# gardiens/EOGS2

Measured on AMD Instinct MI355X. Metric: rasterizer fwd+bwd throughput @1M Gaussians/1024^2 (train iters/s with 1 render/iter), higher is better.
Workload: dtype f32; 1 GPU; 1048576 Gaussians x 1024x1024 x 5 channels, opacity=init, 1 view per GPU, fwd+bwd; gaussians=1048576, height=1024, width=1024, num_rendered=4236528, list_entries=1681274, list_block_px=8, parallelism=view-dp1

## Files before the change

eogs2_amd/csrc/common.h:

```cpp
#pragma once
#include <hip/hip_runtime.h>
#include <stdint.h>
#include <stddef.h>
#include <stdlib.h>

#include "eogs_rast.h"
#include "eogs_loss.h"
#include "eogs_optim.h"
#include "eogs_resample.h"
#include "eogs_knn.h"
#include "eogs_shade.h"
#include "eogs_reg.h"
#include "eogs_pan.h"
#include "eogs_density.h"
#include "eogs_step.h"
#include "eogs_monitor.h"
#include "eogs_tsdf.h"
#include "eogs_dsm.h"

#define NCH EOGS_RAST_CHANNELS
#define TILE EOGS_RAST_TILE
#define SUBX 8
#define SUBY 8
#define PPL (SUBX * SUBY / 64)
// ... 131 lines not shown
#define EOGS_DEPTH_SWITCH 0
#define MACRO_KEY_BITS 16
static_assert(BLOCK_BIG * BLOCK_BIG <= 16, "the sub-mask lives in the upper 16 bits of the sort key");

template <int MACRO, class Emit>
__device__ inline void walk_macro_row(uint32_t kind, unsigned long long m, const SpanParams& sp, int sx0, int sy0, int sx1,
                                      int sy1, int MY, Emit&& emit) {
  const int sw = sx1 - sx0;
  int c0[MACRO], c1[MACRO];
  unsigned long long w[MACRO];
  int lo = 0x7FFFFFFF, hi = -1;
#pragma unroll
  for (int dy = 0; dy < MACRO; dy++) {
    const int fy = MY * MACRO + dy;
    c0[dy] = c1[dy] = 0;
    w[dy] = 0ull;
    if (fy < sy0 || fy >= sy1) continue;
    if (kind == BK_MASK) {
      w[dy] = (m >> ((fy - sy0) * sw)) & (sw >= 64 ? ~0ull : ((1ull << sw) - 1ull));
      if (w[dy]) {
        lo = min(lo, sx0 + (int)__builtin_ctzll(w[dy]));
        hi = max(hi, sx0 + 63 - (int)__builtin_clzll(w[dy]));
      }
    } else {
      if (kind == BK_SPANS) row_span(sp, fy, sx0, sx1, c0[dy], c1[dy]);
      else { c0[dy] = sx0; c1[dy] = sx1; }
      if (c1[dy] > c0[dy]) {
        lo = min(lo, c0[dy]);
        hi = max(hi, c1[dy] - 1);
      }
    }
  }
  if (hi < 0) return;
  for (int MX = lo / MACRO; MX <= hi / MACRO; MX++) {
    const int X0 = MX * MACRO;
    uint32_t sub = 0;
#pragma unroll
    for (int dy = 0; dy < MACRO; dy++) {
      uint32_t nib;
      if (kind == BK_MASK) {
        const int off = X0 - sx0;
        nib = (uint32_t)((off >= 0 ? (w[dy] >> off) : (w[dy] << (-off))) & ((1ull << MACRO) - 1ull));
      } else {
        const int a = max(c0[dy], X0) - X0, b = min(c1[dy], X0 + MACRO) - X0;
        nib = b > a ? (((1u << (b - a)) - 1u) << a) : 0u;
      }
      sub |= nib << (dy * MACRO);
    }
    if (sub) emit(MX, sub);
  }
}

template <int MACRO>
__device__ inline void count_macro_row(uint32_t kind, const SpanParams& sp, int sx0, int sy0, int sx1, int sy1, int MY,
                                       uint32_t& ent, uint32_t& fine) {
  int c0[MACRO], c1[MACRO];
  int lo = 0x7FFFFFFF, hi = -1;
#pragma unroll
  for (int dy = 0; dy < MACRO; dy++) {
    const int fy = MY * MACRO + dy;
    c0[dy] = c1[dy] = 0;
    if (fy < sy0 || fy >= sy1) continue;
    if (kind == BK_SPANS) row_span(sp, fy, sx0, sx1, c0[dy], c1[dy]);
    else { c0[dy] = sx0; c1[dy] = sx1; }
    if (c1[dy] > c0[dy]) {
      lo = min(lo, c0[dy]);
      hi = max(hi, c1[dy] - 1);
    }
  }
  if (hi < 0) return;
  const int B0 = lo / MACRO, B1 = hi / MACRO;
  if (B1 - B0 < 64) {
    unsigned long long m = 0ull;
#pragma unroll
    for (int dy = 0; dy < MACRO; dy++) {
      if (c1[dy] > c0[dy]) {
        const int a = c0[dy] / MACRO - B0, len = (c1[dy] - 1) / MACRO - c0[dy] / MACRO + 1;
        m |= (len >= 64 ? ~0ull : ((1ull << len) - 1ull)) << a;
        fine += (uint32_t)(c1[dy] - c0[dy]);
      }
    }
    ent += (uint32_t)__popcll(m);
  } else {
    walk_macro_row<MACRO>(kind, 0ull, sp, sx0, sy0, sx1, sy1, MY, [&](int, uint32_t sub) {
      ent++;
      fine += (uint32_t)__popc(sub);
    });
  }
}

static inline size_t ws_align(size_t x) { return (x + 255u) & ~(size_t)255u; }

template <typename T>
static inline size_t ws_carve(char* base, size_t off, T*& p, size_t count) {
  off = ws_align(off);
  p = base ? reinterpret_cast<T*>(base + off) : nullptr;
  return off + count * sizeof(T);
}

static inline uint32_t ceil_div_u32(uint64_t a, uint64_t b) { return (uint32_t)((a + b - 1) / b); }

struct GeomWS {
  float4* packed;
  uint4* binfo;
  float4* bext;
  uint32_t* pbkey;
  uint32_t* pblock;
  uint32_t* pblockE;
  uint32_t* bcount;
  uint32_t* bpairs;
  uint32_t* sched;
  uint32_t* where;
  uint32_t* misc;
  float* vmpart;
  uint32_t nblkE;
  size_t bytes;
};

static inline GeomWS geom_layout(char* base, int P) {
  GeomWS g;
  size_t n = (size_t)P, o = 0;
  g.nblkE = ceil_div_u32(n, BLK * EXPAND_ITEMS);
  o = ws_carve(base, o, g.packed, n * 4);
  o = ws_carve(base, o, g.binfo, n * 2);
  o = ws_carve(base, o, g.bext, n * 2);
  o = ws_carve(base, o, g.pblock, (size_t)g.nblkE + 1);
  o = ws_carve(base, o, g.pblockE, (size_t)g.nblkE + 1);
  o = ws_carve(base, o, g.pbkey, (size_t)g.nblkE * 4);
  o = ws_carve(base, o, g.bcount, (size_t)MAX_BLOCKS);
  o = ws_carve(base, o, g.bpairs, (size_t)MAX_BLOCKS);
  o = ws_carve(base, o, g.sched, (size_t)16);
  o = ws_carve(base, o, g.where, (size_t)3 * SCHED_MAX_BLOCKS);
  o = ws_carve(base, o, g.misc, MISC_WORDS);
  o = ws_carve(base, o, g.vmpart, (size_t)g.nblkE * 18);
  g.bytes = ws_align(o) + 256;
  return g;
}

struct SortWS {
  uint4* entA;
  uint4* entB;
  uint32_t* hist;
  uint32_t* histp;
  uint32_t* dtotal;
  uint32_t cap, nblk;
  size_t bytes;
};
static inline uint32_t ent_cap(int P) {
  const uint64_t c = 6ull * (uint64_t)(P < 0 ? 0 : P);
  return c < 4096ull ? 4096u : (c > 0x07FFFFFFull ? 0x07FFFFFFu : (uint32_t)c);
}
static inline SortWS sort_layout(char* base, uint32_t cap) {
  SortWS w;
  size_t o = 0;
  w.cap = cap;
  w.nblk = ceil_div_u32(cap, (uint64_t)SORTE_TILE);
  o = ws_carve(base, o, w.entA, (size_t)cap);
  o = ws_carve(base, o, w.entB, (size_t)cap);
  o = ws_carve(base, o, w.hist, (size_t)SORTE_MAXBINS * (w.nblk ? w.nblk : 1));
  o = ws_carve(base, o, w.histp, (size_t)SORTE_MAXBINS * (w.nblk ? w.nblk : 1));
  o = ws_carve(base, o, w.dtotal, SORTE_MAXBINS);
  w.bytes = ws_align(o) + 256;
  return w;
}

struct BinWS {
  uint2* point_list;
  uint32_t* sorted_keys;
  float* records;
  uint8_t* live;
  uint8_t* qmask;
  SortWS sort;
  int block;
  uint32_t cap_slots, cap_entries;
  size_t bytes;
};

static inline int ceil_log2_u32(uint32_t n) {
  int b = 0;
  while (((uint64_t)1 << b) < n) b++;
  return b;
}

static inline uint32_t nr_slots(int64_t R) { return (uint32_t)((uint64_t)R & 0x7FFFFFFFull); }
static inline uint32_t nr_entries(int64_t R) { return (uint32_t)(((uint64_t)R >> 32) & 0x07FFFFFFull); }
__host__ __device__ inline bool capacity_fits(uint64_t slots, uint64_t entries, uint64_t cap_slots, uint64_t cap_entries) {
  return slots <= cap_slots && entries <= cap_entries;
}
static inline int nr_alt(int64_t R) { return (int)(((uint64_t)R >> 59) & 1ull); }
static inline int nr_shallow(int64_t R) { return (int)(((uint64_t)R >> 60) & 1ull); }
static inline int nr_sorted(int64_t R) { return (int)(((uint64_t)R >> 61) & 1ull); }
static inline int nr_block(int64_t R) { return (((uint64_t)R >> 62) & 1ull) ? BLOCK_BIG : 1; }
static inline int nr_wide(int64_t R) { return (int)(((uint64_t)R >> 31) & 1ull); }
static inline int64_t nr_pack(uint32_t slots, uint32_t entries, int block, int sorted, int wide, int shallow, int alt = 0) {
  return (int64_t)(((uint64_t)(block > 1) << 62) | ((uint64_t)(sorted != 0) << 61) | ((uint64_t)(shallow != 0) << 60) |
                   ((uint64_t)(alt != 0) << 59) | ((uint64_t)(entries & 0x07FFFFFFu) << 32) | ((uint64_t)(wide != 0) << 31) | slots);
}
static inline uint32_t macro_grid_x(int W, int M) { return (uint32_t)(((W + SUBX - 1) / SUBX + M - 1) / M); }
static inline uint32_t macro_grid_y(int H, int M) { return (uint32_t)(((H + SUBY - 1) / SUBY + M - 1) / M); }
static inline void block_sort_geometry(int H, int W, int& passes, int& bits) {
  const uint32_t nb = macro_grid_x(W, BLOCK_BIG) * macro_grid_y(H, BLOCK_BIG);
  const int tb = ceil_log2_u32(nb) < 1 ? 1 : ceil_log2_u32(nb);
  passes = tb <= 12 ? 1 : 2;
  bits = (tb + passes - 1) / passes;
}

static inline BinWS bin_layout(char* base, int H, int W, int64_t R) {
  (void)H; (void)W;
  BinWS b;
  const size_t ne = (size_t)nr_entries(R), nslots = (size_t)nr_slots(R);
  size_t o = 0;
  b.block = nr_block(R);
  b.cap_slots = (uint32_t)nslots;
  b.cap_entries = (uint32_t)ne;
  o = ws_carve(base, o, b.point_list, b.block > 1 ? ne : nslots);
  o = ws_carve(base, o, b.sorted_keys, b.block > 1 ? ne : (size_t)0);
  o = ws_carve(base, o, b.records, nslots * REC);
  o = ws_carve(base, o, b.live, nslots);
  o = ws_carve(base, o, b.qmask, b.block > 1 ? (size_t)0 : nslots);
  b.sort = sort_layout(nullptr, 0);
  if (!nr_sorted(R) && ne) {
    o = ws_align(o);
    b.sort = sort_layout(base ? base + o : nullptr, (uint32_t)ne);
    o += b.sort.bytes;
  }
  b.bytes = ws_align(o) + 256;
  return b;
}

struct ImgWS {
  uint2* ranges;
  float* final_T;
  uint32_t* n_contrib;
  uint4* desc;
  uint32_t sched_lg;
  size_t bytes;
};

static inline ImgWS img_layout(char* base, int H, int W) {
  ImgWS im;
  size_t n = (size_t)H * W, o = 0;
  size_t T = (size_t)macro_grid_x(W, 1) * macro_grid_y(H, 1);
  const uint32_t nblocks = macro_grid_x(W, BLOCK_BIG) * macro_grid_y(H, BLOCK_BIG);
  o = ws_carve(base, o, im.ranges, T);
  o = ws_carve(base, o, im.final_T, n);
  o = ws_carve(base, o, im.n_contrib, n);
  im.desc = nullptr;
  im.sched_lg = 0;
  if (nblocks <= SCHED_MAX_BLOCKS && sched_enabled()) {
    im.sched_lg = sched_capacity(nblocks);
    o = ws_carve(base, o, im.desc, (size_t)8 * 16 * im.sched_lg);
  }
  im.bytes = ws_align(o) + 256;
  return im;
}

static inline char* ws_base(const void* p) {
  return reinterpret_cast<char*>((reinterpret_cast<uintptr_t>(p) + 255u) & ~(uintptr_t)255u);
}

struct FwdPrepArgs {
  int P, H, W;
  const float *means3D, *scales, *rotations, *cov3D_precomp, *opacities, *colors, *viewmatrix;
  float scale_modifier;
  bool antialiasing;
  int* radii;
  bool raw;
  const float* alt_affine;
};
void launch_preprocess_fwd(const FwdPrepArgs& a, const GeomWS& g, hipStream_t s);
void launch_pblock_scan(const GeomWS& g, int P, hipStream_t s);
void launch_entry_sort(const GeomWS& g, const SortWS& w, int P, int H, int W, hipStream_t s);
static inline bool entry_sort_result_in_A(int H, int W) {
  int passes, bits;
  block_sort_geometry(H, W, passes, bits);
  return (passes & 1) == 0;
}
void launch_block_lists(const GeomWS& g, const SortWS& w, const BinWS& b, const ImgWS& im, int P, int H, int W, int64_t R,
                        hipStream_t s);
void launch_render_fwd(const GeomWS& g, const BinWS& b, const ImgWS& im, int P, int H, int W, int64_t R,
                       const float* bg, float* out_color, float* out_invdepth, hipStream_t s);
void launch_render_bwd(const GeomWS& g, const BinWS& b, const ImgWS& im, int P, int H, int W, int64_t R,
                       const float* dL_dcolor, const float* dL_dinvdepth, const float* bg, bool raw, hipStream_t s);
int render_fwd_variant(int block, int64_t R, int P);
int render_bwd_variant(int block, int64_t R, int P);
int render_bwd_noflag_ok(int block, int64_t R, int P);
struct GaussBwdArgs {
  int P, H, W;
  const float *means3D, *scales, *rotations, *cov3D_precomp, *opacities, *viewmatrix, *projmatrix;
  const int* radii;
  float scale_modifier;
  bool antialiasing;
  float *dL_dmeans2D, *dL_dcolors, *dL_dopacity, *dL_dmeans3D, *dL_dcov3D, *dL_dscales, *dL_drotations;
  float *dL_dT_sum, *dL_dvm_mean;
  bool raw;
  const float* alt_affine;
  float* dL_dcolors_lead;
  int lead_cols;
  bool alt_only;
  int noflag_ok;
  int wide;
};
#define GB_WIDE_DEPTH 256.0f
int gaussian_bwd_wide(int64_t R, int P);
void launch_gaussian_bwd(const GaussBwdArgs& a, const GeomWS& g, const BinWS& b, int p_begin, int p_end, hipStream_t s);
void launch_selftest(uint32_t* out, hipStream_t s);

#define LOSS_WIN EOGS_LOSS_WINDOW
struct LossWindow {
  float w[LOSS_WIN];
  float ws, c1, c0;
};
struct LossWS {
  float* partial;
  float* plane_tmp;
  float* maps;
  size_t map_stride;
  int tiles;
  size_t bytes;
};
LossWS loss_layout(char* base, int planes, int H, int W, unsigned mode);
bool loss_grid_fits(int planes, int H);
void launch_loss_fwd(const LossWS& w, int planes, int H, int W, const float* img, const float* gt, unsigned mode,
                     float w_l1, float w_ssim, float bias, float* out, float* plane_sums, hipStream_t s);

void launch_sort_u32(uint32_t* keyA, uint32_t* valA, uint32_t* keyB, uint32_t* valB, uint32_t n, int passes, uint32_t* hist,
                     uint32_t nblk, uint32_t* dtotal, hipStream_t s);
```

eogs2_amd/csrc/preprocess.hip:

```cpp
#include "common.h"
#include "reduce.h"
#include <type_traits>

namespace {

struct Mat3 {
  float m[3][3];
};

__device__ inline Mat3 quat_to_Rm(float r, float x, float y, float z) {
  Mat3 R;
  R.m[0][0] = 1.f - 2.f * (y * y + z * z); R.m[1][0] = 2.f * (x * y - r * z); R.m[2][0] = 2.f * (x * z + r * y);
  R.m[0][1] = 2.f * (x * y + r * z); R.m[1][1] = 1.f - 2.f * (x * x + z * z); R.m[2][1] = 2.f * (y * z - r * x);
  R.m[0][2] = 2.f * (x * z - r * y); R.m[1][2] = 2.f * (y * z + r * x); R.m[2][2] = 1.f - 2.f * (x * x + y * y);
  return R;
}

__device__ inline void cov3d_from_scale_rot(const float s[3], float mod, const float q[4], float c6[6]) {
  Mat3 R = quat_to_Rm(q[0], q[1], q[2], q[3]);
  float sc[3] = {mod * s[0], mod * s[1], mod * s[2]};
  float M[3][3];
#pragma unroll
  for (int i = 0; i < 3; i++)
#pragma unroll
    for (int j = 0; j < 3; j++) M[i][j] = sc[i] * R.m[i][j];
  float S[3][3];
#pragma unroll
  for (int i = 0; i < 3; i++)
#pragma unroll
    for (int j = i; j < 3; j++) S[i][j] = M[0][i] * M[0][j] + M[1][i] * M[1][j] + M[2][i] * M[2][j];
  c6[0] = S[0][0]; c6[1] = S[0][1]; c6[2] = S[0][2]; c6[3] = S[1][1]; c6[4] = S[1][2]; c6[5] = S[2][2];
}

__device__ inline void build_T(const float* __restrict__ vm, int W, int H, float T[2][3]) {
  const float sx = (float)(W / 2.0), sy = (float)(H / 2.0);
#pragma unroll
  for (int k = 0; k < 3; k++) {
    T[0][k] = vm[4 * k + 0] * sx;
    T[1][k] = vm[4 * k + 1] * sy;
  }
}

__device__ inline void cov2d(const float T[2][3], const float c6[6], float& cxx, float& cxy, float& cyy) {
  const float V[3][3] = {{c6[0], c6[1], c6[2]}, {c6[1], c6[3], c6[4]}, {c6[2], c6[4], c6[5]}};
  float A[2][3];
#pragma unroll
  for (int i = 0; i < 2; i++)
#pragma unroll
    for (int l = 0; l < 3; l++) A[i][l] = T[i][0] * V[0][l] + T[i][1] * V[1][l] + T[i][2] * V[2][l];
  cxx = A[0][0] * T[0][0] + A[0][1] * T[0][1] + A[0][2] * T[0][2];
  cxy = A[1][0] * T[0][0] + A[1][1] * T[0][1] + A[1][2] * T[0][2];
  cyy = A[1][0] * T[1][0] + A[1][1] * T[1][1] + A[1][2] * T[1][2];
}

__device__ inline int clampi(int v, int lo, int hi) { return v < lo ? lo : (v > hi ? hi : v); }

__device__ inline void stage_rows3_load(const float* __restrict__ src, size_t row0, int rows, float (&r)[3]) {
  const int t = threadIdx.x, n = rows * 3;
  const float* p = src + row0 * 3;
#pragma unroll
  for (int i = 0; i < 3; i++) {
    const int e = i * BLK + t;
    r[i] = e < n ? p[e] : 0.f;
  }
}
__device__ inline void stage_rows3_store(int rows, const float (&r)[3], float* s_dst) {
  const int t = threadIdx.x, n = rows * 3;
#pragma unroll
  for (int i = 0; i < 3; i++) {
    const int e = i * BLK + t;
    if (e < n) s_dst[e] = r[i];
  }
}

constexpr float SH_C0 = 0.28209479177387814f;

__device__ inline float sigmoidf(float x) { return 1.f / (1.f + expf(-x)); }

__device__ inline float raw_activate(float s[3], float q[4], bool* clamped = nullptr) {
#pragma unroll
  for (int k = 0; k < 3; k++) s[k] = expf(s[k]);
  const float n = sqrtf(q[0] * q[0] + q[1] * q[1] + q[2] * q[2] + q[3] * q[3]);
  if (clamped) *clamped = n < 1e-12f;
  const float inv = 1.f / fmaxf(n, 1e-12f);
#pragma unroll
  for (int k = 0; k < 4; k++) q[k] *= inv;
  return inv;
}

#ifndef GB_COOP
#define GB_COOP 64u
#endif

}

#ifndef EOGS_PP_WAVES
#define EOGS_PP_WAVES 6
#endif
#define PP_ATTR __attribute__((amdgpu_waves_per_eu(EOGS_PP_WAVES, EOGS_PP_WAVES)))
template <bool RAW>
__global__ __launch_bounds__(BLK) PP_ATTR void preprocess_fwd_kernel(
    int P, int H, int W, int gx, int gy,
    const float* __restrict__ means3D, const float* __restrict__ scales, const float* __restrict__ rotations,
    const float* __restrict__ cov3D_precomp, const float* __restrict__ opacities, const float* __restrict__ colors,
    const float* __restrict__ vm, const float* __restrict__ alt, float scale_modifier, int antialiasing,
    int* __restrict__ radii, float4* __restrict__ packed, uint4* __restrict__ binfo, float4* __restrict__ bext,
    uint32_t* __restrict__ pblock,
    uint32_t* __restrict__ pbkey) {
  __shared__ float s_m[3 * BLK];
  __shared__ float s_s[3 * BLK];
  __shared__ float s_c[RAW ? 3 * BLK : 1];
  __shared__ uint32_t s_cnt[BLK / 64];
  const int t = threadIdx.x;
  const size_t row0 = (size_t)blockIdx.x * BLK;
  const int rows = (int)(((size_t)P - row0) < (size_t)BLK ? ((size_t)P - row0) : (size_t)BLK);
  float4 q_pre = make_float4(1.f, 0.f, 0.f, 0.f);
  float op_pre = 0.f;
  {
    float st_m[3], st_s[3] = {0.f, 0.f, 0.f}, st_c[3] = {0.f, 0.f, 0.f};
    stage_rows3_load(means3D, row0, rows, st_m);
    if (scales) stage_rows3_load(scales, row0, rows, st_s);
    if (RAW) stage_rows3_load(colors, row0, rows, st_c);
    if (t < rows) {
      if (!cov3D_precomp) q_pre = reinterpret_cast<const float4*>(rotations)[row0 + t];
      op_pre = opacities[row0 + t];
    }
    stage_rows3_store(rows, st_m, s_m);
    if (scales) stage_rows3_store(rows, st_s, s_s);
    if (RAW) stage_rows3_store(rows, st_c, s_c);
  }
  __syncthreads();

  const size_t idx = row0 + t;
  uint32_t my_tiles = 0, my_entries = 0, key_bits = 0, bkind = BK_RECT, my_err = 0;
  uint32_t op64 = 0;
  uint4 bi0 = make_uint4(0u, 0u, 0u, 0u);
  bool need_count = false;
  uint32_t c_kind = BK_RECT;
  SpanParams c_sp = {};
  int c_sx0 = 0, c_sy0 = 0, c_sx1 = 0, c_sy1 = 0;
  if (t < rows) {
    const float p[3] = {s_m[3 * t], s_m[3 * t + 1], s_m[3 * t + 2]};
    float pv[3];
#pragma unroll
    for (int i = 0; i < 3; i++) pv[i] = vm[i] * p[0] + vm[4 + i] * p[1] + vm[8 + i] * p[2] + vm[12 + i];

    float c6[6];
    if (cov3D_precomp) {
      const float2* c2 = reinterpret_cast<const float2*>(cov3D_precomp + 6 * idx);
      float2 a = c2[0], b = c2[1], c = c2[2];
      c6[0] = a.x; c6[1] = a.y; c6[2] = b.x; c6[3] = b.y; c6[4] = c.x; c6[5] = c.y;
    } else {
      const float4 q = q_pre;
      float s[3] = {s_s[3 * t], s_s[3 * t + 1], s_s[3 * t + 2]};
      float qq[4] = {q.x, q.y, q.z, q.w};
      if (RAW) raw_activate(s, qq);
      cov3d_from_scale_rot(s, scale_modifier, qq, c6);
    }
    float T[2][3];
    build_T(vm, W, H, T);
    float cx, cy, cz;
    cov2d(T, c6, cx, cy, cz);

    const float h_var = 0.3f;
    const float det_cov = cx * cz - cy * cy;
    cx += h_var;
    cz += h_var;
    const float det = cx * cz - cy * cy;
    float hcs = 1.0f;
    if (antialiasing) hcs = sqrtf(fmaxf(0.000025f, det_cov / det));

    int radius = 0;
    if (det != 0.0f) {
      const float det_inv = 1.f / det;
      const float mid = 0.5f * (cx + cz);
      const float root = sqrtf(fmaxf(0.1f, mid * mid - det));
      const float lambda1 = mid + root, lambda2 = mid - root;
      const float my_radius = ceilf(3.f * sqrtf(fmaxf(lambda1, lambda2)));
      const float px = (float)((((double)pv[0] + 1.0) * W - 1.0) * 0.5);
      const float py = (float)((((double)pv[1] + 1.0) * H - 1.0) * 0.5);
      const int r = (int)my_radius;
      const int x0 = clampi((int)((px - r) / TILE), 0, gx);
      const int y0 = clampi((int)((py - r) / TILE), 0, gy);
      const int x1 = clampi((int)((px + r + TILE - 1) / TILE), 0, gx);
      const int y1 = clampi((int)((py + r + TILE - 1) / TILE), 0, gy);
      const int area = (x1 - x0) * (y1 - y0);
      if (area != 0) {
        radius = r;
        const float d = (float)(200.0 - (double)pv[2]);
        if (d < 0) my_err = 0x80000000u;
        const float op_in = RAW ? sigmoidf(op_pre) : op_pre;
        const float ca = cz * det_inv, cb = -cy * det_inv, cc = cx * det_inv, op = op_in * hcs;
        op64 = (uint32_t)(fminf(fmaxf(op, 0.f), 1.f) * 64.f + 0.5f);
        const int gsx = (W + SUBX - 1) / SUBX, gsy = (H + SUBY - 1) / SUBY;
        int sx0 = FX * x0, sy0 = FY * y0;
        int sx1 = FX * x1 < gsx ? FX * x1 : gsx, sy1 = FY * y1 < gsy ? FY * y1 : gsy;
        const float tau = 2.f * __logf(255.f * op);
        const float tau_m = tau + 1e-3f * (1.f + fabsf(tau));
        bool any = true;
        if (op < 1.f / 255.f) {
          any = false;
        } else if (tau_m >= 0.f && tau_m < 3.0e38f) {
          const float ex = __builtin_amdgcn_sqrtf(tau_m * cx) * 1.001f + 1e-2f, ey = __builtin_amdgcn_sqrtf(tau_m * cz) * 1.001f + 1e-2f;
          const float fx0 = floorf((px - ex) * (1.f / SUBX)), fx1 = floorf((px + ex) * (1.f / SUBX)) + 1.f;
          const float fy0 = floorf((py - ey) * (1.f / SUBY)), fy1 = floorf((py + ey) * (1.f / SUBY)) + 1.f;
          if (fx0 > (float)sx0) sx0 = (int)fminf(fx0, (float)sx1);
          if (fy0 > (float)sy0) sy0 = (int)fminf(fy0, (float)sy1);
          if (fx1 < (float)sx1) sx1 = (int)fmaxf(fx1, (float)sx0);
          if (fy1 < (float)sy1) sy1 = (int)fmaxf(fy1, (float)sy0);
        }
        const int sw = sx1 - sx0, sh = sy1 - sy0;
        unsigned long long m = 0ull;
        uint32_t kind = BK_RECT;
        SpanParams sp = {};
        if (!any || sw <= 0 || sh <= 0) {
          my_tiles = 0;
        } else if (sw * sh <= MASK_MAX_SUBTILES) {
          kind = BK_MASK;
          const int bx0 = sx0 / BLOCK_BIG, by0 = sy0 / BLOCK_BIG, bw = (sx1 - 1) / BLOCK_BIG - bx0 + 1;
          unsigned long long blocks = 0ull;
          if (tau_m >= 0.f && tau_m < 3.0e38f && ca * cc - cb * cb > 0.f) {
            const SpanParams spm = span_params(px, py, ca, cb, cc, tau_m);
            for (int sy = sy0; sy < sy1; sy++) {
              int c0, c1;
              row_span(spm, sy, sx0, sx1, c0, c1);
              if (c1 > c0) {
                const unsigned long long run = (c1 - c0 >= 64 ? ~0ull : ((1ull << (c1 - c0)) - 1ull)) << (c0 - sx0);
                m |= run << ((sy - sy0) * sw);
                const int b0 = c0 / BLOCK_BIG - bx0, b1 = (c1 - 1) / BLOCK_BIG - bx0;
                blocks |= (((1ull << (b1 - b0 + 1)) - 1ull) << b0) << ((sy / BLOCK_BIG - by0) * bw);
              }
            }
          } else {
            const float b_c = cb / cc, b_a = cb / ca;
            for (int sy = sy0; sy < sy1; sy++)
              for (int sx = sx0; sx < sx1; sx++) {
                const float bx = (float)(sx * SUBX), by = (float)(sy * SUBY);
                if (block_hit(px, py, ca, cb, cc, b_c, b_a, tau_m, bx, by, bx + (SUBX - 1), by + (SUBY - 1))) {
                  m |= 1ull << ((sy - sy0) * sw + (sx - sx0));
                  blocks |= 1ull << ((sy / BLOCK_BIG - by0) * bw + (sx / BLOCK_BIG - bx0));
                }
              }
          }
          my_tiles = (uint32_t)__popcll(m);
          my_entries = (uint32_t)__popcll(blocks);
        } else if (tau_m >= 0.f && tau_m < 3.0e38f && ca * cc - cb * cb > 0.f) {
          kind = BK_SPANS;
          sp = span_params(px, py, ca, cb, cc, tau_m);
          my_tiles = 1;
        } else {
          my_tiles = (uint32_t)(sw * sh);
        }
        if (my_tiles && kind != BK_MASK) {
          need_count = true;
          c_kind = kind; c_sp = sp; c_sx0 = sx0; c_sy0 = sy0; c_sx1 = sx1; c_sy1 = sy1;
          if (kind == BK_SPANS) {
            bext[2 * idx] = make_float4(sp.gx, sp.gy, sp.ex, sp.ey);
            bext[2 * idx + 1] = make_float4(sp.boa, sp.boc, sp.ta, sp.da);
          }
        }
        bkind = kind;
        if (my_tiles) {
          const float L2E = 1.4426950408889634f;
          float f[NCH];
          if (RAW) {
#pragma unroll
            for (int k = 0; k < 3; k++) f[k] = s_c[3 * t + k] * SH_C0 + 0.5f;
            f[3] = alt[0] * p[0] + alt[1] * p[1] + alt[2] * p[2] + alt[3];
            f[4] = 1.f;
          } else {
#pragma unroll
            for (int k = 0; k < NCH; k++) f[k] = colors[NCH * idx + k];
          }
          packed[4 * idx + 0] = make_float4(px, py, ca * (-0.5f * L2E), cb * L2E);
          packed[4 * idx + 1] = make_float4(cc * (-0.5f * L2E), op, f[0], f[1]);
          packed[4 * idx + 2] = make_float4(f[2], f[3], f[4], 1.f / d);
          bi0 = make_uint4((uint32_t)sx0 | ((uint32_t)sx1 << 16), (uint32_t)sy0 | ((uint32_t)sy1 << 16), (uint32_t)m,
                           (uint32_t)(m >> 32));
          key_bits = __float_as_uint(d);
        }
      }
    }
    radii[idx] = radius;
  }
  {
    const int lane = t & 63;
    const int my0 = c_sy0 / BLOCK_BIG, my1 = (c_sy1 - 1) / BLOCK_BIG;
    const uint32_t mrows = need_count ? (uint32_t)(my1 - my0 + 1) : 0u;
    const bool tall = mrows >= 4u;
    const uint32_t walk_cost = wave_max_u32_dpp(mrows);
    const uint32_t coop_cost = wave_sum_u32_dpp(tall ? 2u : 0u) + 3u;
    const bool together = coop_cost < walk_cost;
    uint32_t ent = 0, fine = 0;
    unsigned long long big = __ballot(tall && together);
    while (big) {
      const int src = __builtin_ctzll(big);
      big &= big - 1ull;
      SpanParams gs;
      gs.gx = __shfl(c_sp.gx, src, 64); gs.gy = __shfl(c_sp.gy, src, 64); gs.ex = __shfl(c_sp.ex, src, 64);
      gs.ey = __shfl(c_sp.ey, src, 64); gs.boa = __shfl(c_sp.boa, src, 64); gs.boc = __shfl(c_sp.boc, src, 64);
      gs.ta = __shfl(c_sp.ta, src, 64); gs.da = __shfl(c_sp.da, src, 64);
      const uint32_t gk = __shfl(c_kind, src, 64);
      const int gx0 = __shfl(c_sx0, src, 64), gy0 = __shfl(c_sy0, src, 64), gx1 = __shfl(c_sx1, src, 64), gy1 = __shfl(c_sy1, src, 64);
      uint32_t ne = 0, nf = 0;
      for (int MY = gy0 / BLOCK_BIG + lane; MY <= (gy1 - 1) / BLOCK_BIG; MY += 64)
        count_macro_row<BLOCK_BIG>(gk, gs, gx0, gy0, gx1, gy1, MY, ne, nf);
      ne = wave_sum_u32_dpp(ne);
      nf = wave_sum_u32_dpp(nf);
      if (lane == src) { ent = ne; fine = nf; }
    }
    if (need_count) {
      if (!(tall && together))
        for (int MY = my0; MY <= my1; MY++) count_macro_row<BLOCK_BIG>(c_kind, c_sp, c_sx0, c_sy0, c_sx1, c_sy1, MY, ent, fine);
      my_tiles = fine;
      my_entries = ent;
    }
  }
  const uint32_t inc = wave_incl_scan_u32(my_tiles);
  const int lane = t & 63;
  if (lane == 63) s_cnt[t >> 6] = inc;
  __syncthreads();
  const uint32_t w0 = s_cnt[0], w1 = s_cnt[1], w2 = s_cnt[2], w3 = s_cnt[3];
  const int w = t >> 6;
  const uint32_t pre = (w > 0 ? w0 : 0u) + (w > 1 ? w1 : 0u) + (w > 2 ? w2 : 0u);
  if (t < rows) {
    binfo[idx] = bi0;
    binfo[(size_t)P + idx] = make_uint4(my_tiles, pre + inc - my_tiles, key_bits, bkind | (my_entries << 2));
  }
  __shared__ uint32_t s_k[5][BLK / 64];
  uint32_t kmax = my_tiles ? key_bits : 0u, knmin = my_tiles ? ~key_bits : 0u, esum = my_tiles ? my_entries : 0u;
  const unsigned long long o64 = (unsigned long long)my_tiles * op64;
  uint32_t osum = o64 > 0x7FFFFFull ? 0x7FFFFFu : (uint32_t)o64;
  kmax = wave_max_u32_dpp(kmax);
  knmin = wave_max_u32_dpp(knmin);
  esum = wave_sum_u32_dpp(esum);
  osum = wave_sum_u32_dpp(osum);
  my_err = wave_or_u32_dpp(my_err);
  if (lane == 0) { s_k[0][w] = kmax; s_k[1][w] = knmin; s_k[2][w] = esum; s_k[3][w] = osum; s_k[4][w] = my_err; }
  __syncthreads();
  if (t == 0) {
    pblock[blockIdx.x] = w0 + w1 + w2 + w3;
    uint32_t a = s_k[0][0], b = s_k[1][0], e = s_k[2][0], ow = s_k[3][0], er = s_k[4][0];
    for (int i = 1; i < BLK / 64; i++) {
      a = s_k[0][i] > a ? s_k[0][i] : a;
      b = s_k[1][i] > b ? s_k[1][i] : b;
      e += s_k[2][i];
      ow += s_k[3][i];
      er |= s_k[4][i];
    }
    pbkey[4 * blockIdx.x] = a;
    pbkey[4 * blockIdx.x + 1] = b;
    pbkey[4 * blockIdx.x + 2] = e;
    pbkey[4 * blockIdx.x + 3] = ow | er;
  }
}

void launch_preprocess_fwd(const FwdPrepArgs& a, const GeomWS& g, hipStream_t s) {
  const int gx = (a.W + TILE - 1) / TILE, gy = (a.H + TILE - 1) / TILE;
  const uint32_t nblk = ceil_div_u32((uint64_t)a.P, BLK);
  auto* kern = a.raw ? preprocess_fwd_kernel<true> : preprocess_fwd_kernel<false>;
  hipLaunchKernelGGL(kern, dim3(nblk), dim3(BLK), 0, s, a.P, a.H, a.W, gx, gy, a.means3D, a.scales, a.rotations,
                     a.cov3D_precomp, a.opacities, a.colors, a.viewmatrix, a.alt_affine, a.scale_modifier,
                     (int)a.antialiasing, a.radii, g.packed, g.binfo, g.bext, g.pblock, g.pbkey);
}


template <bool RAW, bool ALT, int WIDE>
__global__ __launch_bounds__(BLK) __attribute__((amdgpu_waves_per_eu(WIDE ? (ALT ? 5 : 4) : 6, WIDE ? (ALT ? 5 : 4) : 8))) void gaussian_bwd_kernel(
    int P, int H, int W,
    const float* __restrict__ means3D, const float* __restrict__ scales, const float* __restrict__ rotations,
    const float* __restrict__ cov3D_precomp, const float* __restrict__ opacities, const float* __restrict__ vm,
    const float* __restrict__ proj, const float* __restrict__ alt, const int* __restrict__ radii, float scale_modifier, int antialiasing,
    const uint4* __restrict__ binfo, const uint32_t* __restrict__ pblock, const float* __restrict__ records,
    const uint8_t* __restrict__ live,
    float* __restrict__ dL_dmeans2D, float* __restrict__ dL_dcolors, float* __restrict__ dL_dopacity,
    float* __restrict__ dL_dmeans3D, float* __restrict__ dL_dcov3D, float* __restrict__ dL_dscales,
    float* __restrict__ dL_drotations, bool want_T, bool want_vm, float* __restrict__ vmpart, uint32_t blk0,
    float* __restrict__ dL_dcolors_lead, int lead_cols, const uint32_t* __restrict__ misc, uint32_t cap_slots,
    uint32_t cap_entries, int noflag_ok) {
  __shared__ float s_m[3 * BLK];
  __shared__ float s_s[3 * BLK];
  __shared__ float s_red[BLK / 64][18];
  __shared__ float s_coop[11][BLK];
  constexpr uint32_t GB_DIRECT = WIDE == 2 ? 8u : 4u;
  constexpr bool GB_WIDE = WIDE != 0;
  const bool fits = misc[MISC_TOTAL_HI] == 0u && misc[MISC_MACRO_HI] == 0u && misc[MISC_TOTAL_LO] <= cap_slots &&
                    misc[MISC_MACRO_LO] <= cap_entries;
  const float opw = (float)misc[MISC_OPW_LO] + 4294967296.0f * (float)misc[MISC_OPW_HI];
  const float ntiles8 = (float)((W + SUBX - 1) / SUBX) * (float)((H + SUBY - 1) / SUBY);
  const uint32_t dlim = opw > 64.0f * 60.0f * ntiles8 ? 1u : GB_DIRECT;
  const bool noflag = (noflag_ok & 1) != 0 && ((noflag_ok & 2) != 0 || noflag_scene(misc[MISC_OPW_LO], misc[MISC_OPW_HI], W, H));
  const int t = threadIdx.x;
  const uint32_t blk = blk0 + blockIdx.x;
  const size_t row0 = (size_t)blk * BLK;
  const int rows = (int)(((size_t)P - row0) < (size_t)BLK ? ((size_t)P - row0) : (size_t)BLK);
  const size_t idx = row0 + t;
  float vmsum[18];
#pragma unroll
  for (int k = 0; k < 18; k++) vmsum[k] = 0.f;
  float acc[12];
#pragma unroll
  for (int k = 0; k < 12; k++) acc[k] = 0.f;
  bool visible = false;
  float4 rot_in = make_float4(1.f, 0.f, 0.f, 0.f);
  float op_raw = 0.f;
  float st_m[3], st_s[3] = {0.f, 0.f, 0.f};
  stage_rows3_load(means3D, row0, rows, st_m);
  if (scales) stage_rows3_load(scales, row0, rows, st_s);

  int radius_in = 0;
  uint4 bi1 = make_uint4(0u, 0u, 0u, 0u);
  uint32_t pb = 0;
  if (t < rows) {
    radius_in = radii[idx];
    bi1 = binfo[(size_t)P + idx];
    pb = pblock[blk];
    if (!cov3D_precomp) rot_in = reinterpret_cast<const float4*>(rotations)[idx];
    if (RAW || antialiasing) op_raw = opacities[idx];
  }
  visible = t < rows && radius_in > 0;
  const uint32_t n_all = (visible && fits) ? bi1.x : 0u;
  const bool is_big = n_all > GB_COOP;

  {
    const int lane = t & 63;
    unsigned long long big = __builtin_amdgcn_ballot_w64(is_big);
    while (big) {
      const int src = (int)__builtin_ctzll(big);
      big &= big - 1ull;
      const uint32_t n = (uint32_t)__builtin_amdgcn_readlane((int)n_all, src);
      const uint32_t s0 = (uint32_t)__builtin_amdgcn_readlane((int)(pb + bi1.y), src);
      constexpr int RQc = (ALT ? REC_ALT : REC) / 4;
      const float4* r4c = reinterpret_cast<const float4*>(records);
      float part[11];
#pragma unroll
      for (int k = 0; k < 11; k++) part[k] = 0.f;
#pragma unroll 2
      for (uint32_t q0 = 0; q0 < n; q0 += 64u) {
        const uint32_t q = q0 + (uint32_t)lane;
        const bool lv = q < n && (noflag || live[s0 + q] != 0);
        const uint32_t qq = q < n ? q : 0u;
        const float4 ra = r4c[rec_q((size_t)s0 + qq, 0, RQc)];
        const float4 rb = r4c[rec_q((size_t)s0 + qq, 1, RQc)];
        float3 rc = make_float3(0.f, 0.f, 0.f);
        if (!ALT) rc = reinterpret_cast<const float3*>(r4c + rec_q((size_t)s0 + qq, 2, RQc))[0];
        if (lv) {
          part[0] += ra.x; part[1] += ra.y; part[2] += ra.z; part[5] += ra.w;
          part[3] += rb.x; part[4] += rb.y;
          if (ALT) {
            part[9] += rb.z;
          } else {
            part[6] += rb.z; part[7] += rb.w;
            part[8] += rc.x; part[9] += rc.y; part[10] += rc.z;
          }
        }
      }
#pragma unroll
      for (int k = 0; k < 11; k++) {
        const float tot = wave_sum_dpp(part[k]);
        if (lane == 0) s_coop[k][(t & ~63) + src] = tot;
      }
    }
  }

  {
    if (visible) {
      const uint32_t n = is_big ? 0u : n_all;
      const size_t s0 = (size_t)pb + bi1.y;
      constexpr int RQ = (ALT ? REC_ALT : REC) / 4;
      const float4* r4 = reinterpret_cast<const float4*>(records);
      uint32_t q_first = 0;
      if (n <= dlim) {
        float4 ra[GB_DIRECT], rb[GB_DIRECT];
        float3 rc[GB_DIRECT];
        bool lv[GB_DIRECT];
        static_assert(GB_DIRECT == 4u || GB_DIRECT == 8u, "one or two dwords of flags");
        unsigned long long fl4 = 0x0101010101010101ull;
        if (!noflag && n) __builtin_memcpy(&fl4, live + s0, GB_DIRECT);
#pragma unroll
        for (uint32_t u = 0; u < GB_DIRECT; u++) {
          const uint32_t qq = u < n ? u : 0u;
          lv[u] = false;
          if (u < n) {
            lv[u] = ((uint32_t)(fl4 >> (8u * u)) & 0xFFu) != 0u;
            ra[u] = r4[rec_q(s0 + qq, 0, RQ)];
            rb[u] = r4[rec_q(s0 + qq, 1, RQ)];
            if (!ALT) rc[u] = reinterpret_cast<const float3*>(r4 + rec_q(s0 + qq, 2, RQ))[0];
          }
        }
#pragma unroll
        for (uint32_t u = 0; u < GB_DIRECT; u++) {
          if (lv[u]) {
            acc[0] += ra[u].x; acc[1] += ra[u].y; acc[2] += ra[u].z; acc[5] += ra[u].w;
            acc[3] += rb[u].x; acc[4] += rb[u].y;
            if (ALT) {
              acc[9] += rb[u].z;
            } else {
              acc[6] += rb[u].z; acc[7] += rb[u].w;
              acc[8] += rc[u].x; acc[9] += rc[u].y; acc[10] += rc[u].z;
            }
          }
        }
        q_first = n;
      }
      for (uint32_t q0 = q_first; q0 < n; q0 += 32) {
        const uint32_t m_n = n - q0 < 32u ? n - q0 : 32u;
        uint32_t m = 0;
        const uint32_t all = m_n >= 32u ? 0xFFFFFFFFu : (1u << m_n) - 1u;
        if (noflag) {
          m = all;
        } else {
#pragma unroll 2
          for (uint32_t q = 0; q < m_n; q += 4) {
            uint32_t f;
            __builtin_memcpy(&f, live + s0 + q0 + q, 4);
            m |= ((f & 1u) | ((f >> 7) & 2u) | ((f >> 14) & 4u) | ((f >> 21) & 8u)) << q;
          }
          m &= all;
        }
        auto trip = [&](auto widthc) {
          constexpr int NW = decltype(widthc)::value;
          uint32_t q[NW];
          bool have[NW];
#pragma unroll
          for (int u = 0; u < NW; u++) {
            have[u] = m != 0u;
            q[u] = have[u] ? q0 + (uint32_t)__builtin_ctz(m) : q0;
            m &= m - 1u;
          }
          float4 ra[NW], rb[NW];
          float3 rc[NW];
#pragma unroll
          for (int u = 0; u < NW; u++) {
            if (NW > 4 && u >= 4) {
              if (have[u]) {
                ra[u] = r4[rec_q(s0 + q[u], 0, RQ)];
                rb[u] = r4[rec_q(s0 + q[u], 1, RQ)];
                if (!ALT) rc[u] = reinterpret_cast<const float3*>(r4 + rec_q(s0 + q[u], 2, RQ))[0];
              }
              continue;
            }
            const uint32_t qq = have[u] ? q[u] : q[0];
            ra[u] = r4[rec_q(s0 + qq, 0, RQ)];
            rb[u] = r4[rec_q(s0 + qq, 1, RQ)];
            if (!ALT) rc[u] = reinterpret_cast<const float3*>(r4 + rec_q(s0 + qq, 2, RQ))[0];
          }
#pragma unroll
          for (int u = 0; u < NW; u++) {
            if (have[u]) {
              acc[0] += ra[u].x; acc[1] += ra[u].y; acc[2] += ra[u].z; acc[5] += ra[u].w;
              acc[3] += rb[u].x; acc[4] += rb[u].y;
              if (ALT) {
                acc[9] += rb[u].z;
              } else {
                acc[6] += rb[u].z; acc[7] += rb[u].w;
                acc[8] += rc[u].x; acc[9] += rc[u].y; acc[10] += rc[u].z;
              }
            }
          }
        };
        while (m) {
          if (GB_WIDE && __builtin_amdgcn_ballot_w64(__popc(m) > 4) != 0ull) trip(std::integral_constant<int, 8>{});
          else trip(std::integral_constant<int, 4>{});
        }
      }
    }
  }
  stage_rows3_store(rows, st_m, s_m);
  if (scales) stage_rows3_store(rows, st_s, s_s);
  __syncthreads();
  if (is_big) {
#pragma unroll
    for (int k = 0; k < 11; k++) acc[k] = s_coop[k][t];
  }
  if (t < rows) {
    const float gxn = acc[0], gyn = acc[1];
    float dop = acc[5];
    float dcov[6] = {0.f, 0.f, 0.f, 0.f, 0.f, 0.f};
    float dmean3[3] = {0.f, 0.f, 0.f};
    float dscale[3] = {0.f, 0.f, 0.f};
    float dq[4] = {0.f, 0.f, 0.f, 0.f};
    const float m[3] = {s_m[3 * t], s_m[3 * t + 1], s_m[3 * t + 2]};

    if (visible) {
      float c6[6];
      float q[4] = {1.f, 0.f, 0.f, 0.f};
      float s3[3] = {0.f, 0.f, 0.f};
      float q_inv = 1.f, op_in = 0.f;
      bool q_clamped = false;
      if (RAW || antialiasing) op_in = RAW ? sigmoidf(op_raw) : op_raw;
      if (cov3D_precomp) {
        const float2* c2 = reinterpret_cast<const float2*>(cov3D_precomp + 6 * idx);
        float2 a = c2[0], b = c2[1], c = c2[2];
        c6[0] = a.x; c6[1] = a.y; c6[2] = b.x; c6[3] = b.y; c6[4] = c.x; c6[5] = c.y;
      } else {
        const float4 qq = rot_in;
        q[0] = qq.x; q[1] = qq.y; q[2] = qq.z; q[3] = qq.w;
        s3[0] = s_s[3 * t]; s3[1] = s_s[3 * t + 1]; s3[2] = s_s[3 * t + 2];
        if (RAW) q_inv = raw_activate(s3, q, &q_clamped);
        cov3d_from_scale_rot(s3, scale_modifier, q, c6);
      }
      float T[2][3];
      build_T(vm, W, H, T);
      float c_xx, c_xy, c_yy;
      cov2d(T, c6, c_xx, c_xy, c_yy);
      const float dLc[3] = {acc[2], acc[3], acc[4]};

      const float h_var = 0.3f;
      float d_inside_root = 0.f;
      if (antialiasing) {
        const float det_cov = c_xx * c_yy - c_xy * c_xy;
        c_xx += h_var;
        c_yy += h_var;
        const float det_p = c_xx * c_yy - c_xy * c_xy;
        const float hcs = sqrtf(fmaxf(0.000025f, det_cov / det_p));
        const float d_hcs = dop * op_in;
        dop = dop * hcs;
        d_inside_root = (det_cov / det_p) <= 0.000025f ? 0.f : d_hcs / (2 * hcs);
      } else {
        c_xx += h_var;
        c_yy += h_var;
      }
      float dxx = 0.f, dxy = 0.f, dyy = 0.f;
      if (antialiasing) {
        const float x = c_xx, y = c_yy, z = c_xy, w = h_var;
        const float sqv = w * w + w * (x + y) + x * y - z * z;
        const float denom_f = d_inside_root / (sqv * sqv);
        dxx = w * (w * y + y * y + z * z) * denom_f;
        dyy = w * (w * x + x * x + z * z) * denom_f;
        dxy = -2.f * w * z * (w + x + y) * denom_f;
      }
      const float denom = c_xx * c_yy - c_xy * c_xy;
      const float denom2inv = 1.0f / ((denom * denom) + 0.0000001f);
      if (denom2inv != 0) {
        dxx += denom2inv * (-c_yy * c_yy * dLc[0] + 2 * c_xy * c_yy * dLc[1] + (denom - c_xx * c_yy) * dLc[2]);
        dyy += denom2inv * (-c_xx * c_xx * dLc[2] + 2 * c_xx * c_xy * dLc[1] + (denom - c_xx * c_yy) * dLc[0]);
        dxy += denom2inv * 2 * (c_xy * c_yy * dLc[0] - (denom + 2 * c_xy * c_xy) * dLc[1] + c_xx * c_xy * dLc[2]);
        dcov[0] = (T[0][0] * T[0][0] * dxx + T[0][0] * T[1][0] * dxy + T[1][0] * T[1][0] * dyy);
        dcov[3] = (T[0][1] * T[0][1] * dxx + T[0][1] * T[1][1] * dxy + T[1][1] * T[1][1] * dyy);
        dcov[5] = (T[0][2] * T[0][2] * dxx + T[0][2] * T[1][2] * dxy + T[1][2] * T[1][2] * dyy);
        dcov[1] = 2 * T[0][0] * T[0][1] * dxx + (T[0][0] * T[1][1] + T[0][1] * T[1][0]) * dxy + 2 * T[1][0] * T[1][1] * dyy;
        dcov[2] = 2 * T[0][0] * T[0][2] * dxx + (T[0][0] * T[1][2] + T[0][2] * T[1][0]) * dxy + 2 * T[1][0] * T[1][2] * dyy;
        dcov[4] = 2 * T[0][2] * T[0][1] * dxx + (T[0][1] * T[1][2] + T[0][2] * T[1][1]) * dxy + 2 * T[1][1] * T[1][2] * dyy;
      }
      if (want_T) {
        const float V[3][3] = {{c6[0], c6[1], c6[2]}, {c6[1], c6[3], c6[4]}, {c6[2], c6[4], c6[5]}};
        float TV[2][3];
#pragma unroll
        for (int r = 0; r < 2; r++)
#pragma unroll
          for (int k = 0; k < 3; k++) TV[r][k] = T[r][0] * V[k][0] + T[r][1] * V[k][1] + T[r][2] * V[k][2];
#pragma unroll
        for (int k = 0; k < 3; k++) {
          vmsum[k] = 2 * TV[0][k] * dxx + TV[1][k] * dxy;
          vmsum[3 + k] = 2 * TV[1][k] * dyy + TV[0][k] * dxy;
        }
      }
      dmean3[0] = proj[0] * gxn + proj[1] * gyn;
      dmean3[1] = proj[4] * gxn + proj[5] * gyn;
      dmean3[2] = proj[8] * gxn + proj[9] * gyn;

      if (!cov3D_precomp) {
        const Mat3 R = quat_to_Rm(q[0], q[1], q[2], q[3]);
        const float s[3] = {scale_modifier * s3[0], scale_modifier * s3[1], scale_modifier * s3[2]};
        float M[3][3];
#pragma unroll
        for (int a = 0; a < 3; a++)
#pragma unroll
          for (int c = 0; c < 3; c++) M[a][c] = s[a] * R.m[a][c];
        const float dS[3][3] = {{dcov[0], 0.5f * dcov[1], 0.5f * dcov[2]},
                                {0.5f * dcov[1], dcov[3], 0.5f * dcov[4]},
                                {0.5f * dcov[2], 0.5f * dcov[4], dcov[5]}};
        float dM[3][3];
#pragma unroll
        for (int a = 0; a < 3; a++)
#pragma unroll
          for (int c = 0; c < 3; c++)
            dM[a][c] = (2.0f * M[a][0]) * dS[0][c] + (2.0f * M[a][1]) * dS[1][c] + (2.0f * M[a][2]) * dS[2][c];
#pragma unroll
        for (int k = 0; k < 3; k++) dscale[k] = R.m[k][0] * dM[k][0] + R.m[k][1] * dM[k][1] + R.m[k][2] * dM[k][2];
        float D[3][3];
#pragma unroll
        for (int a = 0; a < 3; a++)
#pragma unroll
          for (int c = 0; c < 3; c++) D[a][c] = dM[a][c] * s[a];
        const float r = q[0], x = q[1], y = q[2], z = q[3];
        dq[0] = 2 * z * (D[0][1] - D[1][0]) + 2 * y * (D[2][0] - D[0][2]) + 2 * x * (D[1][2] - D[2][1]);
        dq[1] = 2 * y * (D[1][0] + D[0][1]) + 2 * z * (D[2][0] + D[0][2]) + 2 * r * (D[1][2] - D[2][1]) - 4 * x * (D[2][2] + D[1][1]);
        dq[2] = 2 * x * (D[1][0] + D[0][1]) + 2 * r * (D[2][0] - D[0][2]) + 2 * z * (D[1][2] + D[2][1]) - 4 * y * (D[2][2] + D[0][0]);
        dq[3] = 2 * r * (D[0][1] - D[1][0]) + 2 * x * (D[2][0] + D[0][2]) + 2 * y * (D[1][2] + D[2][1]) - 4 * z * (D[1][1] + D[0][0]);
      }
      if (RAW) {
#pragma unroll
        for (int k = 0; k < 3; k++) dscale[k] *= s3[k];
        const float dot = q_clamped ? 0.f : q[0] * dq[0] + q[1] * dq[1] + q[2] * dq[2] + q[3] * dq[3];
#pragma unroll
        for (int k = 0; k < 4; k++) dq[k] = (dq[k] - q[k] * dot) * q_inv;
        dop *= op_in * (1.f - op_in);
#pragma unroll
        for (int k = 0; k < 3; k++) dmean3[k] += alt[k] * acc[9];
      }
    }
    dL_dmeans2D[3 * idx] = gxn; dL_dmeans2D[3 * idx + 1] = gyn; dL_dmeans2D[3 * idx + 2] = 0.f;
    if (RAW) {
#pragma unroll
      for (int ch = 0; ch < 3; ch++) dL_dcolors[3 * idx + ch] = SH_C0 * acc[6 + ch];
    } else {
#pragma unroll
      for (int ch = 0; ch < NCH; ch++) dL_dcolors[NCH * idx + ch] = acc[6 + ch];
    }
    if (dL_dcolors_lead) {
#pragma unroll
      for (int ch = 0; ch < NCH; ch++)
        if (ch < lead_cols) dL_dcolors_lead[(size_t)lead_cols * idx + ch] = (RAW ? SH_C0 : 1.f) * acc[6 + ch];
    }
    dL_dopacity[idx] = dop;
#pragma unroll
    for (int k = 0; k < 3; k++) dL_dmeans3D[3 * idx + k] = dmean3[k];
    if (dL_dcov3D) {
#pragma unroll
      for (int k = 0; k < 6; k++) dL_dcov3D[6 * idx + k] = dcov[k];
    }
    if (dL_dscales) {
#pragma unroll
      for (int k = 0; k < 3; k++) dL_dscales[3 * idx + k] = dscale[k];
    }
    if (dL_drotations) reinterpret_cast<float4*>(dL_drotations)[idx] = make_float4(dq[0], dq[1], dq[2], dq[3]);

    if (want_vm) {
#pragma unroll
      for (int a = 0; a < 3; a++) {
        vmsum[6 + 3 * a + 0] = m[a] * gxn;
        vmsum[6 + 3 * a + 1] = m[a] * gyn;
      }
      vmsum[15] = gxn;
      vmsum[16] = gyn;
    }
  }

  if (want_T || want_vm) {
#pragma unroll
    for (int k = 0; k < 18; k++) {
      float v = wave_sum(vmsum[k]);
      if ((t & 63) == 0) s_red[t >> 6][k] = v;
    }
    __syncthreads();
    if (t < 18) {
      float v = 0.f;
#pragma unroll
      for (int w = 0; w < BLK / 64; w++) v += s_red[w][t];
      vmpart[(size_t)blk * 18 + t] = v;
    }
  }
}

__global__ __launch_bounds__(BLK) void camera_sum_kernel(const float* __restrict__ vmpart, uint32_t nblk,
                                                         float* __restrict__ dL_dT_sum, float* __restrict__ dL_dvm_mean) {
  __shared__ float s_p[14][18];
  const int t = threadIdx.x;
  if (t < 14 * 18) {
    const int c = t % 18, r0 = t / 18;
    float v = 0.f;
    for (uint32_t r = r0; r < nblk; r += 14) v += vmpart[(size_t)r * 18 + c];
    s_p[r0][c] = v;
  }
  __syncthreads();
  if (t < 18) {
    float v = 0.f;
#pragma unroll
    for (int r = 0; r < 14; r++) v += s_p[r][t];
    if (t < 6) {
      if (dL_dT_sum) dL_dT_sum[t] = v;
    } else if (dL_dvm_mean) {
      const int k = t - 6;
      if (k < 9) dL_dvm_mean[k] = (k % 3) < 2 ? v : 0.f;
      else dL_dvm_mean[k] = (k - 9) < 2 ? v : 0.f;
    }
  }
}

int gaussian_bwd_wide(int64_t R, int P) {
  static const int forced = [] {
    const char* e = getenv("EOGS_GB_WIDE");
    return e ? atoi(e) : -1;
  }();
  if (forced >= 0) return forced > 2 ? 2 : forced;
  if (!nr_shallow(R) || P <= 0) return 0;
  return (double)nr_slots(R) >= 6.0 * (double)P ? 2 : 1;
}

void launch_gaussian_bwd(const GaussBwdArgs& a, const GeomWS& g, const BinWS& b, int p_begin, int p_end, hipStream_t s) {
  const uint32_t nblk_all = ceil_div_u32((uint64_t)a.P, BLK);
  const uint32_t blk0 = (uint32_t)p_begin / BLK, nblk = ceil_div_u32((uint64_t)(p_end - p_begin), BLK);
  const bool want_T = a.dL_dT_sum != nullptr, want_vm = a.dL_dvm_mean != nullptr;
  using Kern = decltype(&gaussian_bwd_kernel<false, false, 0>);
  static Kern const table[3][2][2] = {
      {{gaussian_bwd_kernel<false, false, 0>, gaussian_bwd_kernel<false, true, 0>}, {gaussian_bwd_kernel<true, false, 0>, gaussian_bwd_kernel<true, true, 0>}},
      {{gaussian_bwd_kernel<false, false, 1>, gaussian_bwd_kernel<false, true, 1>}, {gaussian_bwd_kernel<true, false, 1>, gaussian_bwd_kernel<true, true, 1>}},
      {{gaussian_bwd_kernel<false, false, 2>, gaussian_bwd_kernel<false, true, 2>}, {gaussian_bwd_kernel<true, false, 2>, gaussian_bwd_kernel<true, true, 2>}}};
  Kern kern = table[a.wide < 0 ? 0 : (a.wide > 2 ? 2 : a.wide)][a.raw ? 1 : 0][a.alt_only ? 1 : 0];
  if (nblk)
    hipLaunchKernelGGL(kern, dim3(nblk), dim3(BLK), 0, s, a.P, a.H, a.W, a.means3D, a.scales, a.rotations,
                       a.cov3D_precomp, a.opacities, a.viewmatrix, a.projmatrix, a.alt_affine, a.radii, a.scale_modifier,
                       (int)a.antialiasing, g.binfo, g.pblock, b.records, b.live, a.dL_dmeans2D, a.dL_dcolors, a.dL_dopacity,
                       a.dL_dmeans3D, a.dL_dcov3D, a.dL_dscales, a.dL_drotations, want_T, want_vm, g.vmpart, blk0,
                       a.dL_dcolors_lead, a.lead_cols, g.misc, b.cap_slots, b.cap_entries, a.noflag_ok);
  if ((want_T || want_vm) && p_end == a.P)
    hipLaunchKernelGGL(camera_sum_kernel, dim3(1), dim3(BLK), 0, s, g.vmpart, nblk_all, a.dL_dT_sum, a.dL_dvm_mean);
}
```

Measured before the change: 1728 views/s.

## Stream per-block gradient records through LDS ring with async global_load_lds

Adds a streaming variant of the per-Gaussian backward kernel that loads each block's contiguous range of per-pixel gradient records in fixed-size chunks into a double-buffered LDS ring using global_load_lds, plus liveness flags. Each thread then accumulates its own records from LDS rather than doing scattered global loads. The goal is coalesced, overlapped record fetches for large scenes. It is picked by default when P is at least 2^19 and the scene is not wide. The cost is more LDS use, a barrier per chunk, and inline asm that manipulates m0.

```diff
diff --git a/eogs2_amd/csrc/common.h b/eogs2_amd/csrc/common.h
--- a/eogs2_amd/csrc/common.h
+++ b/eogs2_amd/csrc/common.h
@@ -457,6 +457,8 @@
   int wide;
 };
 #define GB_WIDE_DEPTH 256.0f
+#define GB_STREAM_MIN_P (1 << 19)
+#define GB_CHUNK 256u
 int gaussian_bwd_wide(int64_t R, int P);
 void launch_gaussian_bwd(const GaussBwdArgs& a, const GeomWS& g, const BinWS& b, int p_begin, int p_end, hipStream_t s);
 void launch_selftest(uint32_t* out, hipStream_t s);
diff --git a/eogs2_amd/csrc/preprocess.hip b/eogs2_amd/csrc/preprocess.hip
--- a/eogs2_amd/csrc/preprocess.hip
+++ b/eogs2_amd/csrc/preprocess.hip
@@ -91,6 +91,24 @@
 #ifndef GB_COOP
 #define GB_COOP 64u
 #endif
+
+template <bool STREAM, bool ALT>
+struct GaussBwdLds {
+  float m[3 * BLK], s[3 * BLK];
+  __device__ float* rows_m() { return m; }
+  __device__ float* rows_s() { return s; }
+};
+template <bool ALT>
+struct GaussBwdLds<true, ALT> {
+  static constexpr uint32_t RQ = (ALT ? REC_ALT : REC) / 4;
+  static constexpr uint32_t CH4 = GB_CHUNK * RQ;
+  static_assert(CH4 % BLK == 0 && GB_CHUNK == 4 * 64, "a stage is whole 16-byte-per-lane loads of the workgroup; its flags one dword per lane of a wave");
+  static_assert(2 * CH4 * 4 >= 6 * BLK, "the rows of means3D and scales fit in the ring");
+  alignas(16) float ring[2 * CH4 * 4];
+  uint32_t live[2][GB_CHUNK / 4];
+  __device__ float* rows_m() { return ring; }
+  __device__ float* rows_s() { return ring + 3 * BLK; }
+};
 
 }
 
@@ -378,12 +396,15 @@
     float* __restrict__ dL_drotations, bool want_T, bool want_vm, float* __restrict__ vmpart, uint32_t blk0,
     float* __restrict__ dL_dcolors_lead, int lead_cols, const uint32_t* __restrict__ misc, uint32_t cap_slots,
     uint32_t cap_entries, int noflag_ok) {
-  __shared__ float s_m[3 * BLK];
-  __shared__ float s_s[3 * BLK];
+  constexpr bool STREAM = WIDE == 3;
+  __shared__ GaussBwdLds<STREAM, ALT> s_l;
+  float* const s_m = s_l.rows_m();
+  float* const s_s = s_l.rows_s();
   __shared__ float s_red[BLK / 64][18];
   __shared__ float s_coop[11][BLK];
   constexpr uint32_t GB_DIRECT = WIDE == 2 ? 8u : 4u;
   constexpr bool GB_WIDE = WIDE != 0;
+  static_assert(WIDE >= 0 && WIDE <= 3, "narrow, two wide builds, the streaming build");
   const bool fits = misc[MISC_TOTAL_HI] == 0u && misc[MISC_MACRO_HI] == 0u && misc[MISC_TOTAL_LO] <= cap_slots &&
                     misc[MISC_MACRO_LO] <= cap_entries;
   const float opw = (float)misc[MISC_OPW_LO] + 4294967296.0f * (float)misc[MISC_OPW_HI];
@@ -410,11 +431,15 @@
 
   int radius_in = 0;
   uint4 bi1 = make_uint4(0u, 0u, 0u, 0u);
-  uint32_t pb = 0;
+  uint32_t pb = 0, pe = 0;
+  if (STREAM) {
+    pb = pblock[blk];
+    pe = pblock[blk + 1];
+  }
   if (t < rows) {
     radius_in = radii[idx];
     bi1 = binfo[(size_t)P + idx];
-    pb = pblock[blk];
+    if (!STREAM) pb = pblock[blk];
     if (!cov3D_precomp) rot_in = reinterpret_cast<const float4*>(rotations)[idx];
     if (RAW || antialiasing) op_raw = opacities[idx];
   }
@@ -463,7 +488,7 @@
     }
   }
 
-  {
+  if constexpr (!STREAM) {
     if (visible) {
       const uint32_t n = is_big ? 0u : n_all;
       const size_t s0 = (size_t)pb + bi1.y;
@@ -565,6 +590,81 @@
         }
       }
     }
+  } else {
+    (void)dlim;
+    constexpr uint32_t RQ = GaussBwdLds<true, ALT>::RQ, CH4 = GaussBwdLds<true, ALT>::CH4;
+    const uint32_t L = (fits && pe > pb) ? pe - pb : 0u;
+    const uint32_t nch = (L + GB_CHUNK - 1u) / GB_CHUNK;
+    const float4* rsrc = reinterpret_cast<const float4*>(records) + (size_t)pb * RQ;
+    const uint32_t last4 = L * RQ - 1u;
+    uint32_t fl_next = 0;
+    auto fetch = [&](uint32_t k) {
+      const uint32_t st = k & 1u;
+#pragma unroll
+      for (uint32_t i = 0; i < CH4 / BLK; i++) {
+        const uint32_t j = k * CH4 + i * BLK + (uint32_t)t;
+        const float4* src = rsrc + (j < last4 ? j : last4);
+        const uint32_t dst = __builtin_amdgcn_readfirstlane(
+            (int)(uint32_t)(uintptr_t)(__attribute__((address_space(3))) float*)(s_l.ring + 4u * (st * CH4 + i * BLK + ((uint32_t)t & ~63u))));
+        uint32_t keep;
+        asm volatile("s_mov_b32 %0, m0\n\ts_mov_b32 m0, %2\n\ts_nop 0\n\tglobal_load_lds_dwordx4 %1, off\n\ts_mov_b32 m0, %0"
+                     : "=&s"(keep) : "v"(src), "s"(dst) : "memory");
+      }
+      if (!noflag && t < (int)(GB_CHUNK / 4u)) {
+        const uint32_t o = k * GB_CHUNK + 4u * (uint32_t)t;
+        __builtin_memcpy(&fl_next, live + (size_t)pb + (o < L ? o : L), 4);
+      }
+    };
+    auto publish_flags = [&](uint32_t k) {
+      if (!noflag && t < (int)(GB_CHUNK / 4u)) s_l.live[k & 1u][t] = fl_next;
+    };
+    if (nch) {
+      fetch(0u);
+      publish_flags(0u);
+    }
+    const uint32_t n = is_big ? 0u : n_all;
+    const uint32_t rel0 = bi1.y;
+    for (uint32_t k = 0; k < nch; k++) {
+      asm volatile("s_waitcnt vmcnt(0)" ::: "memory");
+      __syncthreads();
+      if (k + 1u < nch) fetch(k + 1u);
+      const uint32_t c0 = k * GB_CHUNK;
+      const uint32_t lo = rel0 > c0 ? rel0 : c0;
+      const uint32_t hi = rel0 + n < c0 + GB_CHUNK ? rel0 + n : c0 + GB_CHUNK;
+      const float4* rg = reinterpret_cast<const float4*>(s_l.ring) + (k & 1u) * CH4;
+      const uint8_t* lf = reinterpret_cast<const uint8_t*>(s_l.live[k & 1u]);
+      for (uint32_t q = lo; q < hi; q += 4u) {
+        float4 ra[4], rb[4], rc[4];
+        uint32_t fl[4];
+#pragma unroll
+        for (uint32_t u = 0; u < 4u; u++) {
+          const uint32_t r = (q + u < hi ? q + u : q) - c0;
+          fl[u] = noflag ? 1u : (uint32_t)lf[r];
+          ra[u] = rg[r * RQ];
+          rb[u] = rg[r * RQ + 1u];
+          rc[u] = ALT ? rb[u] : rg[r * RQ + (ALT ? 1u : 2u)];
+        }
+#pragma unroll
+        for (uint32_t u = 0; u < 4u; u++) {
+          asm volatile("" : "+v"(ra[u].x), "+v"(rb[u].x), "+v"(rc[u].x), "+v"(fl[u]));
+        }
+#pragma unroll
+        for (uint32_t u = 0; u < 4u; u++) {
+          if (q + u < hi && fl[u] != 0u) {
+            acc[0] += ra[u].x; acc[1] += ra[u].y; acc[2] += ra[u].z; acc[5] += ra[u].w;
+            acc[3] += rb[u].x; acc[4] += rb[u].y;
+            if (ALT) {
+              acc[9] += rb[u].z;
+            } else {
+              acc[6] += rb[u].z; acc[7] += rb[u].w;
+              acc[8] += rc[u].x; acc[9] += rc[u].y; acc[10] += rc[u].z;
+            }
+          }
+        }
+      }
+      if (k + 1u < nch) publish_flags(k + 1u);
+    }
+    __syncthreads();
   }
   stage_rows3_store(rows, st_m, s_m);
   if (scales) stage_rows3_store(rows, st_s, s_s);
@@ -784,9 +884,10 @@
     const char* e = getenv("EOGS_GB_WIDE");
     return e ? atoi(e) : -1;
   }();
-  if (forced >= 0) return forced > 2 ? 2 : forced;
+  if (forced >= 0) return forced > 3 ? 3 : forced;
   if (!nr_shallow(R) || P <= 0) return 0;
-  return (double)nr_slots(R) >= 6.0 * (double)P ? 2 : 1;
+  if ((double)nr_slots(R) >= 6.0 * (double)P) return 2;
+  return P >= GB_STREAM_MIN_P ? 3 : 1;
 }
 
 void launch_gaussian_bwd(const GaussBwdArgs& a, const GeomWS& g, const BinWS& b, int p_begin, int p_end, hipStream_t s) {
@@ -794,11 +895,12 @@
   const uint32_t blk0 = (uint32_t)p_begin / BLK, nblk = ceil_div_u32((uint64_t)(p_end - p_begin), BLK);
   const bool want_T = a.dL_dT_sum != nullptr, want_vm = a.dL_dvm_mean != nullptr;
   using Kern = decltype(&gaussian_bwd_kernel<false, false, 0>);
-  static Kern const table[3][2][2] = {
+  static Kern const table[4][2][2] = {
       {{gaussian_bwd_kernel<false, false, 0>, gaussian_bwd_kernel<false, true, 0>}, {gaussian_bwd_kernel<true, false, 0>, gaussian_bwd_kernel<true, true, 0>}},
       {{gaussian_bwd_kernel<false, false, 1>, gaussian_bwd_kernel<false, true, 1>}, {gaussian_bwd_kernel<true, false, 1>, gaussian_bwd_kernel<true, true, 1>}},
-      {{gaussian_bwd_kernel<false, false, 2>, gaussian_bwd_kernel<false, true, 2>}, {gaussian_bwd_kernel<true, false, 2>, gaussian_bwd_kernel<true, true, 2>}}};
-  Kern kern = table[a.wide < 0 ? 0 : (a.wide > 2 ? 2 : a.wide)][a.raw ? 1 : 0][a.alt_only ? 1 : 0];
+      {{gaussian_bwd_kernel<false, false, 2>, gaussian_bwd_kernel<false, true, 2>}, {gaussian_bwd_kernel<true, false, 2>, gaussian_bwd_kernel<true, true, 2>}},
+      {{gaussian_bwd_kernel<false, false, 3>, gaussian_bwd_kernel<false, true, 3>}, {gaussian_bwd_kernel<true, false, 3>, gaussian_bwd_kernel<true, true, 3>}}};
+  Kern kern = table[a.wide < 0 ? 0 : (a.wide > 3 ? 3 : a.wide)][a.raw ? 1 : 0][a.alt_only ? 1 : 0];
   if (nblk)
     hipLaunchKernelGGL(kern, dim3(nblk), dim3(BLK), 0, s, a.P, a.H, a.W, a.means3D, a.scales, a.rotations,
                        a.cov3D_precomp, a.opacities, a.viewmatrix, a.projmatrix, a.alt_affine, a.radii, a.scale_modifier,
```

Result: faster. 1763 views/s, median of 6 (+2.1%).
